# snap-research/MMVID

Measured on AMD Instinct MI355X. Metric: video-tokens/sec training step, 8-frame 128px text-to-video, higher is better.
Workload: dtype bf16

## Files before the change

include/mmvid_hip.h:

```cpp
#ifndef MMVID_HIP_H
#define MMVID_HIP_H
#include <stdint.h>
#ifdef __cplusplus
extern "C" {
#endif

const char* mmvid_last_error(void);
int mmvid_abi_version(void);
int mmvid_device_count(void);

int mmvid_vq_sqnorm(const float* codebook, int n, int dim, float* ee, void* stream);
int mmvid_vq_argmin_l2(const float* z, const float* codebook, const float* ee, int64_t rows, int n, int dim,
                       int64_t* idx, float* dmin, void* stream);
int mmvid_gather_rows(const float* table, int64_t table_rows, const int64_t* idx, int64_t rows, int dim,
                      float* out_f32, void* out_bf16, void* stream);

int mmvid_gemm_bf16(int a_kmajor, int b_kmajor, int M, int N, int K, const void* A, int64_t lda, const void* B,
                    int64_t ldb, int batch, int64_t strideA, int64_t strideB, int64_t strideC, int splitk,
                    float alpha, const float* bias, const float* residual, int64_t ldr, const void* dact_pre,
                    void* save_pre, int64_t ldp, int act, int accumulate, float* out_f32, void* out_bf16,
                    int64_t ldc, float* out_colsum,
                    void* stream);

int mmvid_decode_trace(void* dev_buf);
int mmvid_decode_persistent_trace(void* dev_buf);

int mmvid_gemm_bf16_dw(int64_t M, int N, int K, const void* dY, int64_t ldy, const void* X, int64_t ldx, int splitk,
                       float* workspace, float* dW, int accumulate, void* stream);
int mmvid_gemm_dw_pick_splitk(int64_t M, int N, int K);
typedef struct {
    int N, K;
    const void* dY;
    int64_t ldy, strideY;
    const void* X;
    int64_t ldx, strideX;
    float* const* dW_list;
} mmvid_dw_kind_t;
int mmvid_gemm_bf16_dw_multi(int64_t M, int nkinds, const mmvid_dw_kind_t* kinds, int groups, int accumulate, void* stream);
int mmvid_gemm_bf16_dw_grouped(int64_t M, int N, int K, const void* dY, int64_t ldy, int64_t strideY, const void* X, int64_t ldx,
                               int64_t strideX, int groups, float* const* dW_list, int accumulate, void* stream);
double mmvid_gemm_dw_multi_fill(int nkinds, const mmvid_dw_kind_t* kinds, int groups);

int mmvid_layernorm_fwd(const float* x, int64_t ldx, int64_t rows, int E, const float* w, const float* b, float eps,
                        void* y_bf16, float* y_f32, int64_t ldy, float* mean, float* rstd, void* stream);
int mmvid_layernorm_bwd(const float* dy, int64_t lddy, const float* x, int64_t ldx, const float* mean,
                        const float* rstd, const float* w, int64_t rows, int E, float* dx, int64_t lddx,
                        int add_into_dx, void* dx_bf16, float* dw, float* db, float* dx_colsum, void* stream);
int mmvid_layernorm_bwd_ws(const float* dy, int64_t lddy, const float* x, int64_t ldx, const float* mean,
                           const float* rstd, const float* w, int64_t rows, int E, float* dx, int64_t lddx,
                           int add_into_dx, void* dx_bf16, float* dw, float* db, float* dx_colsum, float* workspace,
                           int64_t workspace_floats, void* stream);
int mmvid_layernorm_bwd_ex(const void* dy, int dy_is_bf16, int64_t lddy, const float* x, int64_t ldx, const float* mean,
                           const float* rstd, const float* w, int64_t rows, int E, float* dx, int64_t lddx, int add_into_dx,
                           void* dx_bf16, float* dw, float* db, float* dx_colsum, float* workspace, int64_t workspace_floats,
                           void* stream);
typedef struct {
    const float* partial;
    float *dw, *db, *dx_colsum;
} mmvid_ln_reduce_t;
int mmvid_layernorm_bwd_partial(const void* dy, int dy_is_bf16, int64_t lddy, const float* x, int64_t ldx, const float* mean,
                                const float* rstd, const float* w, int64_t rows, int E, float* dx, int64_t lddx, int add_into_dx,
                                void* dx_bf16, int want_dw, int want_db, int want_colsum, float* workspace,
                                int64_t workspace_floats, int* blocks_out, void* stream);
int mmvid_layernorm_bwd_reduce_multi(int n, const mmvid_ln_reduce_t* items, int blocks, int E, void* stream);
int mmvid_groupnorm_swish_nhwc(const void* x, int x_is_bf16, int N, int64_t hw, int C, const float* w,
                               const float* b, float eps, int swish, float* stats_scratch, int partial_blocks,
                               void* y_bf16, float* y_f32, void* stream);

int mmvid_attention_fwd(const void* qkv, int64_t ld, int B, int L, int H, int E, float scale, int mask_mode, int r0,
                        int c0, int r1, int c1, void* out, int64_t ldo, float* lse2, void* stream);
int mmvid_attention_bwd(const void* qkv, int64_t ld, const void* O, int64_t ldo, const void* dO, int64_t lddo,
                        const float* lse2, float* delta, int B, int L, int H, int E, float scale, int mask_mode,
                        int r0, int c0, int r1, int c1, void* dqkv, int64_t ldg, void* stream);
int mmvid_attention_bwd_bias(const void* qkv, int64_t ld, const void* O, int64_t ldo, const void* dO, int64_t lddo,
// ... 342 lines not shown
```

mmvid_amd/_lib.py:

```python
import ctypes
import os
from ctypes import POINTER, Structure, c_char_p, c_float, c_int, c_int32, c_int64, c_uint8, c_uint64, c_void_p

HERE = os.path.dirname(os.path.abspath(__file__))
LIB_PATH = os.environ.get('MMVID_LIB') or os.path.join(HERE, 'libmmvid_hip.so')

P = c_void_p
I, I64, F, U64 = c_int, c_int64, c_float, c_uint64


class TowerLayer(Structure):
    _fields_ = [(n, P) for n in (
        'ln1_w', 'ln1_b', 'ln2_w', 'ln2_b', 'in_w', 'in_b', 'out_w', 'out_b', 'fc_w', 'fc_b', 'pj_w', 'pj_b',
        'g_ln1_w', 'g_ln1_b', 'g_ln2_w', 'g_ln2_b', 'g_in_w', 'g_in_b', 'g_out_w', 'g_out_b', 'g_fc_w', 'g_fc_b',
        'g_pj_w', 'g_pj_b')]


class TowerCfg(Structure):
    _fields_ = [('B', I), ('L', I), ('E', I), ('H', I), ('F', I), ('layers', I), ('mask_mode', I), ('r0', I),
                ('c0', I), ('r1', I), ('c1', I), ('ln_eps', F)]


class DecodeToken(Structure):
    _fields_ = [('tok', c_void_p), ('table', c_void_p), ('table_rows', c_int64), ('pos_rows', c_void_p), ('pos_off', c_int32),
# ... 1 lines not shown
                ('head_w', c_void_p), ('head_b', c_void_p), ('E', c_void_p), ('e_step_stride', c_int64), ('tok_offset', c_int64),
                ('logits_out', c_void_p), ('V', c_int32), ('e_pos0', c_int32), ('lnf_eps', c_float), ('temperature', c_float)]


class PostLnLayer(Structure):
    _fields_ = [(n, P) for n in ('qkv_w', 'qkv_b', 'out_w', 'out_b', 'ln1_w', 'ln1_b', 'fc_w', 'fc_b', 'pj_w', 'pj_b', 'ln2_w', 'ln2_b')]


class PostLnCfg(Structure):
    _fields_ = [('B', I), ('L', I), ('E', I), ('H', I), ('F', I), ('layers', I), ('ln_eps', F)]


class Conv3dCfg(Structure):
    _fields_ = [(n, I) for n in ('N', 'T', 'H', 'W', 'Cin', 'Cout', 'kt', 'kh', 'kw', 'st', 'sh', 'sw', 'pt0', 'pt1', 'ph0', 'ph1',
                                 'pw0', 'pw1', 'relu', 'nseg')] + [('seg_end', I * 3), ('ldo', I * 3), ('c_off', I * 3), ('out', P * 3)]


class VqganOp(Structure):
    _fields_ = [('op', c_int32), ('mode', c_int32), ('N', c_int32), ('H', c_int32), ('W', c_int32), ('C', c_int32),
                ('Cout', c_int32), ('flags', c_int32), ('in0', I64), ('in1', I64), ('in2', I64), ('out_bf16', I64),
                ('out_f32', I64), ('scratch', I64), ('w', P), ('b', P), ('ext_in', P), ('ext_out', P), ('eps', F),
                ('pad', c_int32)]


SIGNATURES = {
    'mmvid_vq_sqnorm': [P, I, I, P, P],
    'mmvid_vq_argmin_l2': [P, P, P, I64, I, I, P, P, P],
    'mmvid_gather_rows': [P, I64, P, I64, I, P, P, P],
    'mmvid_gemm_bf16': [I, I, I, I, I, P, I64, P, I64, I, I64, I64, I64, I, F, P, P, I64, P, P, I64, I, I, P, P, I64, P, P],
    'mmvid_gemm_bf16_dw': [I64, I, I, P, I64, P, I64, I, P, P, I, P],
    'mmvid_gemm_dw_pick_splitk': [I64, I, I],
    'mmvid_gemm_bf16_dw_grouped': [I64, I, I, P, I64, I64, P, I64, I64, I, P, I, P],
    'mmvid_gemm_bf16_dw_multi': [I64, I, P, I, I, P],
    'mmvid_layernorm_fwd': [P, I64, I64, I, P, P, F, P, P, I64, P, P, P],
    'mmvid_layernorm_bwd': [P, I64, P, I64, P, P, P, I64, I, P, I64, I, P, P, P, P, P],
    'mmvid_layernorm_bwd_ws': [P, I64, P, I64, P, P, P, I64, I, P, I64, I, P, P, P, P, P, I64, P],
    'mmvid_layernorm_bwd_partial': [P, I, I64, P, I64, P, P, P, I64, I, P, I64, I, P, I, I, I, P, I64, P, P],
    'mmvid_layernorm_bwd_reduce_multi': [I, P, I, I, P],
    'mmvid_layernorm_bwd_ex': [P, I, I64, P, I64, P, P, P, I64, I, P, I64, I, P, P, P, P, P, I64, P],
    'mmvid_groupnorm_swish_nhwc': [P, I, I, I64, I, P, P, F, I, P, I, P, P, P],
    'mmvid_attention_fwd': [P, I64, I, I, I, I, F, I, I, I, I, I, P, I64, P, P],
    'mmvid_attention_bwd': [P, I64, P, I64, P, I64, P, P, I, I, I, I, F, I, I, I, I, I, P, I64, P],
    'mmvid_attention_bwd_bias': [P, I64, P, I64, P, I64, P, P, I, I, I, I, F, I, I, I, I, I, P, I64, P, P],
    'mmvid_assemble_sequence': [POINTER(P), POINTER(I64), I, P, P, P, I64, I, I, P, P],
    'mmvid_assemble_sequence_bwd': [POINTER(P), POINTER(I64), I, P, P, P, I64, I, I, P, I, P],
    'mmvid_cross_entropy_fwd': [P, I64, P, P, I64, I, P, P, P],
    'mmvid_cross_entropy_bwd': [P, I64, P, P, P, P, I64, I, P, I64, P],
    'mmvid_colsum_bf16': [P, I64, I64, I, P, P],
    'mmvid_grad_sqnorm': [P, I64, P, P],
    'mmvid_adam_step': [P, P, P, P, P, I64, F, F, F, F, F, I, P, F, P, F, P],
    'mmvid_cast_f32_to_bf16': [P, P, I64, P],
    'mmvid_tower_workspace': [POINTER(TowerCfg), POINTER(I64), POINTER(I64)],
    'mmvid_tower_forward': [POINTER(TowerCfg), POINTER(TowerLayer), P, P, P, P, P],
    'mmvid_tower_backward': [POINTER(TowerCfg), POINTER(TowerLayer), P, P, P, P],
    'mmvid_tower_prefill': [POINTER(TowerCfg), POINTER(TowerLayer), P, P, P, I, P, P],
    'mmvid_tower_decode': [POINTER(TowerCfg), POINTER(TowerLayer), P, P, P, I, P, I, P, P],
    'mmvid_tower_decode_fused': [POINTER(TowerCfg), POINTER(TowerLayer), P, P, P, I, P, I, P, P],
    'mmvid_tower_decode_persistent': [POINTER(TowerCfg), POINTER(TowerLayer), P, P, P, I, P, I, I, P, P],
    'mmvid_artv_token_step_persistent': [POINTER(TowerCfg), POINTER(TowerLayer), POINTER(DecodeToken), P, P, I, P, P, P],
    'mmvid_tower_decode_fused_slice': [POINTER(TowerCfg), POINTER(TowerLayer), P, P, P, I, I, P, I, I, P, P],
    'mmvid_gemv_rows': [P, I64, I, I, P, P, F, P, P, I, I, P, I64, I, I, P, I64, P],
    'mmvid_decode_embed': [P, P, I64, P, P, I, I, I, P, P],
    'mmvid_decode_embed_record': [P, P, I64, P, P, I, I, I, P, P, I64, I, P],
    'mmvid_kv_store': [P, I64, I, I, I, P, I, I, P, P],
    'mmvid_attention_decode': [P, I64, P, I, I, I, I, P, I, F, P, I64, P],
    'mmvid_conv2d_nhwc': [I, P, I, I, I, I, P, P, I, P, P, I, P, P, P, P],
# ... 53 lines not shown
    'mmvid_get_option': [c_char_p, POINTER(I)],
    'mmvid_colsum_bf16_det': [P, I64, I64, I, P, P, I64, P],
    'mmvid_cross_entropy_fwd_det': [P, I64, P, P, I64, I, P, P, P, I64, P],
    'mmvid_assemble_sequence_bwd_det': [POINTER(P), POINTER(I64), I, P, P, P, I64, I, I, P, I, P, I64, P],
    'mmvid_gemm_bf16_det': [I, I, I, I, I, P, I64, P, I64, I, I64, I64, I64, I, F, P, P, I64, P, P, I64, I, I, P, P, I64, P, P, I64, P],
    'mmvid_attention_bwd_bias_det': [P, I64, P, I64, P, I64, P, P, I, I, I, I, F, I, I, I, I, I, P, I64, P, P, I64, P],
    'mmvid_device_faults': [P, I],
    'mmvid_pos_table_fwd': [P, I, I, I, P, P],
    'mmvid_pos_table_bwd': [P, I, I, P, P],
    'mmvid_lincomb3': [P, P, P, F, F, F, P, P],
    'mmvid_scale3': [P, F, F, F, P, P, P, P],
    'mmvid_prof_end': [P, P, P, P, I],
    'mmvid_rows_pack': [P, I64, I, P, I, P, P, P],
    'mmvid_rows_merge': [P, I64, I, P, P, I, P],
    'mmvid_clip_patchify': [P, I, I, I, I, I, P, P],
    'mmvid_clip_image_assemble': [P, P, P, P, P, F, I, I, I, P, P],
    'mmvid_clip_text_embed': [P, I, I, P, I64, P, I, P, P, P],
    'mmvid_clip_pool_project': [P, I, I, I, P, P, P, F, P, I, I, P, P],
    'mmvid_clip_pair_scores': [P, P, I, I, I, P, P],
    'mmvid_roberta_embed': [P, P, I, I, P, I64, P, I64, P, P, P, F, I, I64, P, P, P, P],
    'mmvid_attention_fwd_keylen': [P, I64, I, I, I, I, F, P, P, I64, P, P],
    'mmvid_postln_encoder_workspace': [POINTER(PostLnCfg), POINTER(I64)],
    'mmvid_postln_encoder_forward': [POINTER(PostLnCfg), POINTER(PostLnLayer), P, P, P, P, P, P],
    'mmvid_masked_mean_pool': [P, P, I, I, I, P, P],
    'mmvid_conv3d_ndhwc': [POINTER(Conv3dCfg), P, P, P, P],
    'mmvid_maxpool3d_ndhwc': [P, I, I, I, I, I, I, I, I, I, I, I, I, I, I, I, I, I, P, I, I, P],
    'mmvid_i3d_preprocess': [P, I, I, I, I, I, P, P],
    'mmvid_i3d_fold': [P, I, I, P, P],
    'mmvid_i3d_head': [P, I, I, I, P, P, I, P, P],
    'mmvid_frames_to_u8': [P, I64, I, I, P, P],
}
OTHER = {'mmvid_last_error': ([], c_char_p), 'mmvid_abi_version': ([], I), 'mmvid_device_count': ([], I),
         'mmvid_warp_params_bytes': ([], I), 'mmvid_gemm_dw_multi_fill': ([I, P, I], ctypes.c_double),
         'mmvid_tower_decode_persistent_supported': ([POINTER(TowerCfg), I], I),
         'mmvid_tower_decode_persistent_workspace_bytes': ([I], I64),
         'mmvid_colsum_bf16_det_workspace_bytes': ([I64, I], I64), 'mmvid_cross_entropy_fwd_det_workspace_bytes': ([I64], I64),
         'mmvid_assemble_sequence_bwd_det_workspace_bytes': ([I64, I, I, I, POINTER(I64)], I64),
         'mmvid_gemm_bf16_det_workspace_bytes': ([I, I, I, I], I64),
         'mmvid_attention_bwd_bias_det_workspace_bytes': ([I, I, I], I64)}

class DwKind(ctypes.Structure):
    _fields_ = [('N', ctypes.c_int32), ('K', ctypes.c_int32), ('dY', ctypes.c_void_p), ('ldy', ctypes.c_int64), ('strideY', ctypes.c_int64),
                ('X', ctypes.c_void_p), ('ldx', ctypes.c_int64), ('strideX', ctypes.c_int64), ('dW_list', ctypes.c_void_p)]


class LnReduce(ctypes.Structure):
    _fields_ = [('partial', ctypes.c_void_p), ('dw', ctypes.c_void_p), ('db', ctypes.c_void_p), ('dx_colsum', ctypes.c_void_p)]


class PosSegment(ctypes.Structure):
    _fields_ = [('w', ctypes.c_void_p * 3), ('gw', ctypes.c_void_p * 3), ('dst0', ctypes.c_int32), ('rows', ctypes.c_int32),
                ('naxes', ctypes.c_int32), ('src0', ctypes.c_int32), ('d', ctypes.c_int32 * 3), ('pad', ctypes.c_int32)]


ABI_VERSION = 3
_lib = None


class MMVIDError(RuntimeError):
    pass


def load():
    global _lib
    if _lib is None:
        import torch
# ... 81 lines not shown
```

mmvid_amd/csrc/common.h:

```cpp
#pragma once
#include <hip/hip_runtime.h>
#include <stdint.h>
#include <stdio.h>
#include <stdlib.h>
#include <string.h>

typedef uint16_t bf16_t;
typedef __attribute__((ext_vector_type(8))) __bf16 bf16x8_t;
typedef __attribute__((ext_vector_type(8))) _Float16 f16x8_t;
typedef __attribute__((ext_vector_type(4))) float f32x4;
typedef __attribute__((ext_vector_type(16))) float f32x16;

#define MMVID_OK 0
#define MMVID_ERR_ARG 1
#define MMVID_ERR_HIP 2

extern "C" const char* mmvid_last_error();
void mmvid_set_error(const char* fmt, ...);

#define MMVID_REQUIRE(cond, ...)          \
    do {                                  \
        if (!(cond)) {                    \
            mmvid_set_error(__VA_ARGS__); \
            return MMVID_ERR_ARG;         \
// ... 36 lines not shown
template <int CTRL>
__device__ __forceinline__ float dpp_mov(float v) {
    return __builtin_bit_cast(float, __builtin_amdgcn_update_dpp(0, __builtin_bit_cast(int, v), CTRL, 0xf, 0xf, true));
}
__device__ __forceinline__ float wave_sum_fast(float v) {
    v += dpp_mov<0xB1>(v);
    v += dpp_mov<0x4E>(v);
    v += dpp_mov<0x141>(v);
    v += dpp_mov<0x140>(v);
    const uint32_t u = __float_as_uint(v);
    const auto r = __builtin_amdgcn_permlane16_swap(u, u, false, false);
    v = __uint_as_float(r[0]) + __uint_as_float(r[1]);
    const uint32_t w = __float_as_uint(v);
    const auto q = __builtin_amdgcn_permlane32_swap(w, w, false, false);
    return __uint_as_float(q[0]) + __uint_as_float(q[1]);
}
__device__ __forceinline__ float wave_max_fast(float v) {
    v = fmaxf(v, dpp_mov<0xB1>(v));
    v = fmaxf(v, dpp_mov<0x4E>(v));
    v = fmaxf(v, dpp_mov<0x141>(v));
    v = fmaxf(v, dpp_mov<0x140>(v));
    const uint32_t u = __float_as_uint(v);
    const auto r = __builtin_amdgcn_permlane16_swap(u, u, false, false);
    v = fmaxf(__uint_as_float(r[0]), __uint_as_float(r[1]));
    const uint32_t w = __float_as_uint(v);
    const auto q = __builtin_amdgcn_permlane32_swap(w, w, false, false);
    return fmaxf(__uint_as_float(q[0]), __uint_as_float(q[1]));
}

__device__ __forceinline__ void mfma_settle(f32x16& acc) { asm volatile("s_nop 15" : "+v"(acc)); }
__device__ __forceinline__ void mfma_settle(f32x4& acc) { asm volatile("s_nop 15" : "+v"(acc)); }

static inline int cdiv(long a, long b) { return (int)((a + b - 1) / b); }
enum { MMVID_OPT_GRAPHS = 0, MMVID_OPT_DETERMINISTIC = 1, MMVID_OPT_COUNT = 2 };
int mmvid_option(int which);
int mmvid_slab_reduce(const float* slab, int nslabs, int N, float* out, hipStream_t stream);
unsigned long long* mmvid_fault_counters_dev();
```

mmvid_amd/csrc/errors.hip:

```cpp
#include <stdarg.h>

#include "common.h"

static thread_local char g_err[512] = "";

void mmvid_set_error(const char* fmt, ...) {
    va_list ap;
    va_start(ap, fmt);
    vsnprintf(g_err, sizeof(g_err), fmt, ap);
    va_end(ap);
}

extern "C" const char* mmvid_last_error() { return g_err; }

extern "C" int mmvid_abi_version() { return 3; }

extern "C" int mmvid_device_count() {
    int n = 0;
    if (hipGetDeviceCount(&n) != hipSuccess) return 0;
    return n;
}

namespace {
struct Opt {
    const char* name;
    const char* env;
    int dflt, value;
    bool set;
};
Opt g_opts[MMVID_OPT_COUNT] = {{"graphs", "MMVID_GRAPHS", 0, 0, false}, {"deterministic", "MMVID_DETERMINISTIC", 0, 0, false}};
}

int mmvid_option(int which) {
    Opt& o = g_opts[which];
    if (!o.set) {
        const char* e = getenv(o.env);
        o.value = e ? atoi(e) : o.dflt;
        o.set = true;
    }
    return o.value;
}

extern "C" int mmvid_set_option(const char* name, int value) {
    MMVID_REQUIRE(name, "set_option: null name");
    for (int i = 0; i < MMVID_OPT_COUNT; ++i)
        if (strcmp(name, g_opts[i].name) == 0) {
            g_opts[i].value = value, g_opts[i].set = true;
            return MMVID_OK;
        }
    mmvid_set_error("set_option: unknown option '%s' (graphs, deterministic)", name);
    return MMVID_ERR_ARG;
}

extern "C" int mmvid_get_option(const char* name, int* value) {
    MMVID_REQUIRE(name && value, "get_option: null pointer");
    for (int i = 0; i < MMVID_OPT_COUNT; ++i)
        if (strcmp(name, g_opts[i].name) == 0) {
            *value = mmvid_option(i);
            return MMVID_OK;
        }
    mmvid_set_error("get_option: unknown option '%s' (graphs, deterministic)", name);
    return MMVID_ERR_ARG;
}

#include <mutex>
#include <vector>

#include "graphs.h"
#include "prof.h"

namespace {
struct Rec {
    hipEvent_t a, b;
    int cls;
    double flops;
};
bool g_prof_on = false;
int g_prof_stride = 1;
int64_t g_prof_seen[PROF_NCLASS];
std::vector<Rec> g_recs;
std::vector<hipEvent_t> g_pool;
size_t g_pool_next = 0;
std::mutex g_prof_mu;

hipEvent_t pool_get() {
    if (g_pool_next == g_pool.size()) {
        hipEvent_t e;
        (void)hipEventCreate(&e);
        g_pool.push_back(e);
    }
    return g_pool[g_pool_next++];
}
}

// ... 53 lines not shown
```

mmvid_amd/csrc/gemm.hip:

```cpp
#include "../../include/mmvid_hip.h"
#include "gemm_core.h"
#include "prof.h"

namespace {
using namespace mmvid_core;


constexpr int GROUP_MAX = 48;
constexpr int KIND_MAX = 4;
struct GroupKind {
    const unsigned short* A;
    const unsigned short* B;
    long strideA, strideB, lda, ldb;
    int M, N, tiles_n, tiles_m;
    int first;
    int out0;
    int colmajor;
};

struct GemmParams {
    const bf16_t* A;
    const bf16_t* B;
    int M, N, K;
    long lda, ldb;
// ... 553 lines not shown
        tile_origin(tile, bm0, bn0);
        f32x16 acc[2][2];
#pragma unroll
        for (int i = 0; i < 2; ++i)
#pragma unroll
            for (int j = 0; j < 2; ++j)
#pragma unroll
                for (int r = 0; r < 16; ++r) acc[i][j][r] = 0.0f;
        [[maybe_unused]] PreRegs pre_in;
        if constexpr (EPI == 4) pre_load(p, de, bm0, bn0, wm, wn, lane, pre_in);
        k_loop_consumer<AKM, BKM>(smem, nt, wave, lane, wm, wn, acc);
        if constexpr (EPI == 4) {
            pending_fill_dact(p, pre_in, acc, pend, bm0, bn0, wm, wn, lane);
            pending_flush<1>(de, pend);
        } else if constexpr (EPI >= 2) {
            BiasRegs br;
            bias_load(bias_lds, bn0, wn, lane, br);
            pending_fill<NOUT>(p, br, acc, pend, bm0, bn0, wm, wn, lane);
            pending_flush<NOUT>(de, pend);
        } else {
            gemm_epilogue_direct(p, de, bias_lds, acc, bm0, bn0, wm, wn, lane);
        }
    }
}

template <bool AKM, bool BKM, int EPI>
__global__ __launch_bounds__(512 + 64 * mmvid_core::NLOAD, 1) void gemm_bf16_lw_kernel(GemmParams p) {
    gemm_lw_body<AKM, BKM, EPI, false>(p, nullptr);
}
__global__ __launch_bounds__(512 + 64 * mmvid_core::NLOAD, 1) void gemm_bf16_lw_grouped_kernel(GemmParams p, GroupTable gt) {
    gemm_lw_body<true, true, 1, true>(p, &gt);
}

__global__ __launch_bounds__(256) void splitk_reduce_kernel(const float* __restrict__ partial, int splitk, long mn,
                                                            float* __restrict__ out, int accumulate) {
    const long i = ((long)blockIdx.x * 256 + threadIdx.x) * 4;
    if (i >= mn) return;
    float4 a = accumulate ? *reinterpret_cast<const float4*>(out + i) : make_float4(0, 0, 0, 0);
    for (int s = 0; s < splitk; ++s) {
        const float4 v = *reinterpret_cast<const float4*>(partial + (long)s * mn + i);
        a.x += v.x, a.y += v.y, a.z += v.z, a.w += v.w;
    }
    *reinterpret_cast<float4*>(out + i) = a;
}

bool use_big_tile(long M, long N, long zdim) {
    const long blocks = (long)cdiv(M, 256) * cdiv(N, BN) * zdim;
    return M >= 256 && blocks >= 200;
}

constexpr int BIAS_LDS_BYTES = 16384;
bool direct_epilogue_ok(const GemmParams& p) {
    if (p.splitk != 1 || p.partial || p.colsum || p.N > BIAS_LDS_BYTES / 4) return false;
    const long rows = p.M - 1;
    const long ld = p.ldc > p.ldp ? p.ldc : p.ldp;
    const long ldr = p.residual ? p.ldr : 0;
    return (rows * (ld > ldr ? ld : ldr) + p.N) * 4 < (1ll << 31);
}

template <bool AKM, bool BKM, int WM>
void launch_shape(const GemmParams& p, int batch, hipStream_t stream) {
    using S = BlockShape<WM>;
    dim3 grid(cdiv(p.N, BN), cdiv(p.M, S::ROWS), batch * p.splitk);
    GemmParams q = p;
    q.tiles_n = q.tiles_m = 0;
    q.group_n = 0;
// ... 247 lines not shown
        p.A = gt.kinds[0].A, p.B = gt.kinds[0].B;
        p.M = gt.kinds[0].M, p.N = gt.kinds[0].N, p.K = (int)M, p.lda = gt.kinds[0].lda, p.ldb = gt.kinds[0].ldb;
        p.strideA = p.strideB = p.strideC = 0, p.splitk = 1;
        p.bias = nullptr, p.residual = nullptr, p.ldr = 0, p.dact_pre = nullptr, p.save_pre = nullptr, p.ldp = 0;
        p.act = 0, p.accumulate = accumulate, p.alpha = 1.0f;
        p.out_f32 = nullptr, p.out_bf16 = nullptr, p.ldc = gt.kinds[0].N;
        p.partial = nullptr, p.colsum = nullptr, p.colsum_det = 0;
        p.tiles_n = p.tiles_m = 0, p.group_n = 0;
        MmvidProfScope prof(PROF_GEMM_TN, flops, (hipStream_t)stream);
        hipLaunchKernelGGL(gemm_bf16_lw_grouped_kernel, dim3(tiles), dim3(512 + 64 * NLOAD), S::LDS_BYTES + BIAS_LDS_BYTES, (hipStream_t)stream, p, gt);
    }
    MMVID_LAUNCH_CHECK("gemm_bf16_dw_multi");
    return MMVID_OK;
}

extern "C" int mmvid_gemm_bf16_dw_grouped(int64_t M, int N, int K, const void* dY, int64_t ldy, int64_t strideY, const void* X,
                                          int64_t ldx, int64_t strideX, int groups, float* const* dW_list, int accumulate,
                                          void* stream) {
    mmvid_dw_kind_t kd;
    kd.N = N, kd.K = K, kd.dY = dY, kd.ldy = ldy, kd.strideY = strideY, kd.X = X, kd.ldx = ldx, kd.strideX = strideX, kd.dW_list = dW_list;
    return mmvid_gemm_bf16_dw_multi(M, 1, &kd, groups, accumulate, stream);
}

extern "C" double mmvid_gemm_dw_multi_fill(int nkinds, const mmvid_dw_kind_t* kinds, int groups) {
    long tiles = 0;
    for (int k = 0; k < nkinds; ++k) {
        long live = 0;
        for (int g = 0; g < groups; ++g) live += kinds[k].dW_list == nullptr || kinds[k].dW_list[g] != nullptr;
        tiles += (long)cdiv(kinds[k].N, 256) * cdiv(kinds[k].K, BN) * live;
    }
    const long rounds = cdiv(tiles, 256);
    return tiles > 0 ? (double)tiles / (double)(rounds * 256) : 0.0;
}
```

mmvid_amd/csrc/tower.hip:

```cpp
#include "../../include/mmvid_hip.h"
#include "common.h"
#include <vector>

#include "graphs.h"

namespace {

inline int64_t align256(int64_t x) { return (x + 255) & ~(int64_t)255; }
constexpr int kMaxSplitK = 16;
constexpr int kLnBwdBlocks = 512;

struct Dims {
    int B, L, E, H, F, layers;
    int64_t M;
};
Dims dims_of(const mmvid_tower_cfg_t& c) {
    Dims d;
    d.B = c.B, d.L = c.L, d.E = c.E, d.H = c.H, d.F = c.F, d.layers = c.layers;
    d.M = (int64_t)c.B * c.L;
    return d;
}

struct SavedLayer {
    int64_t x_in, x_mid, mean1, rstd1, mean2, rstd2, h1, qkv, o, lse2, h2, pre, act, k_gpj, k_dpre, k_gout, k_dqkv, k_ln1, k_ln2, total;
// ... 140 lines not shown
            }
            x = xin_s;
        }
        float* xnext;
        if (i == d.layers - 1)
            xnext = x_out;
        else if (saved)
            xnext = (float*)((char*)saved + (int64_t)(i + 1) * sl.total + sl.x_in);
        else
            xnext = x_out;
        TRY(mmvid_layernorm_fwd(x, d.E, d.M, d.E, ly.ln1_w, ly.ln1_b, cfg->ln_eps, sv + sl.h1, nullptr, d.E,
                                (float*)(sv + sl.mean1), (float*)(sv + sl.rstd1), stream));
        TRY(linear_fwd(d.M, 3 * d.E, d.E, sv + sl.h1, ly.in_w, ly.in_b, nullptr, nullptr, 0, nullptr, sv + sl.qkv, stream));
        if (kv_cache)
            TRY(mmvid_kv_store(sv + sl.qkv, 3 * d.E, d.B, d.L, d.E, nullptr, 0, kv_lmax,
                               (char*)kv_cache + (int64_t)i * d.B * kv_lmax * 2 * d.E * 2, stream));
        TRY(mmvid_attention_fwd(sv + sl.qkv, 3 * d.E, d.B, d.L, d.H, d.E, scale, cfg->mask_mode, cfg->r0, cfg->c0, cfg->r1,
                                cfg->c1, sv + sl.o, d.E, (float*)(sv + sl.lse2), stream));
        TRY(linear_fwd(d.M, d.E, d.E, sv + sl.o, ly.out_w, ly.out_b, x, nullptr, 0, xmid, nullptr, stream));
        TRY(mmvid_layernorm_fwd(xmid, d.E, d.M, d.E, ly.ln2_w, ly.ln2_b, cfg->ln_eps, sv + sl.h2, nullptr, d.E,
                                (float*)(sv + sl.mean2), (float*)(sv + sl.rstd2), stream));
        TRY(linear_fwd(d.M, d.F, d.E, sv + sl.h2, ly.fc_w, ly.fc_b, nullptr, saved ? sv + sl.pre : nullptr, 1, nullptr,
                       sv + sl.act, stream));
        TRY(linear_fwd(d.M, d.E, d.F, sv + sl.act, ly.pj_w, ly.pj_b, xmid, nullptr, 0, xnext, nullptr, stream));
        x = xnext;
    }
    return MMVID_OK;
}

extern "C" int mmvid_tower_backward(const mmvid_tower_cfg_t* cfg, const mmvid_tower_layer_t* layers, float* g,
                                    void* saved, void* scratch, void* stream) {
    TRY(check_cfg(cfg));
    MMVID_REQUIRE(layers && g && saved && scratch, "tower_backward: null pointer");
    const uint64_t key = tower_key(mmvid_option(MMVID_OPT_DETERMINISTIC) ? 5 : 3, cfg, layers, g, saved, scratch, nullptr, stream);
    return mmvid_run_cached(key, (hipStream_t)stream, [=](hipStream_t s) {
        return tower_backward_enqueue(cfg, layers, g, saved, scratch, (void*)s);
    });
}

static int tower_backward_enqueue(const mmvid_tower_cfg_t* cfg, const mmvid_tower_layer_t* layers, float* g, void* saved,
                                  void* scratch, void* stream) {
    const Dims d = dims_of(*cfg);
    const SavedLayer sl = saved_layout(d);
    const Scratch sc = scratch_layout(d);
    char* scr = (char*)scratch;
    char* keep = (char*)saved;
    struct { int64_t g_pj, d_pre, g_out, dqkv, total; } kl = {sl.k_gpj, sl.k_dpre, sl.k_gout, sl.k_dqkv, sl.total};
    const float scale = 0.125f;
    void* d_h = scr + sc.d_h;
    float* ws = (float*)(scr + sc.splitk_ws);
    void* det_ws = nullptr;
    const int64_t det_bytes = det_slab_bytes(d);
    if (mmvid_option(MMVID_OPT_DETERMINISTIC)) {
        MMVID_REQUIRE(det_bytes <= sc.total - sc.infer, "tower_backward: the deterministic slabs do not fit the scratch arena");
        det_ws = scr + sc.infer;
    }
    const int64_t ln_ws_floats = (int64_t)kLnBwdBlocks * 3 * d.E;
    std::vector<mmvid_ln_reduce_t> ln_items;
    int ln_blocks = 0;
    for (int i = d.layers - 1; i >= 0; --i) {
        const mmvid_tower_layer_t& ly = layers[i];
        const char* sv = (const char*)saved + (int64_t)i * sl.total;
        char* kp = keep + (int64_t)i * kl.total;
        void* g_pj = kp + kl.g_pj;
        if (i == d.layers - 1) {
            TRY(mmvid_cast_f32_to_bf16(g, g_pj, d.M * d.E, stream));
            if (ly.g_pj_b && det_ws) TRY(mmvid_colsum_bf16_det(g_pj, d.E, d.M, d.E, ly.g_pj_b, det_ws, det_bytes, stream));
// ... 24 lines not shown
            int nb = 0;
            TRY(mmvid_layernorm_bwd_partial(d_h, 1, d.E, (const float*)(sv + sl.x_in), d.E, (const float*)(sv + sl.mean1),
                                            (const float*)(sv + sl.rstd1), ly.ln1_w, d.M, d.E, g, d.E, 1,
                                            i > 0 ? (void*)(keep + (int64_t)(i - 1) * kl.total + kl.g_pj) : nullptr, r.dw != nullptr,
                                            r.db != nullptr, r.dx_colsum != nullptr, (float*)(kp + sl.k_ln1), ln_ws_floats, &nb, stream));
            if (r.dw || r.db || r.dx_colsum) ln_items.push_back(r), ln_blocks = nb;
        }
    }
    if (!ln_items.empty()) TRY(mmvid_layernorm_bwd_reduce_multi((int)ln_items.size(), ln_items.data(), ln_blocks, d.E, stream));
    struct Kind {
        int N, K;
        int64_t dy_off, x_off;
        float* mmvid_tower_layer_t::*gw;
    };
    const Kind kinds[4] = {{d.E, d.F, kl.g_pj, sl.act, &mmvid_tower_layer_t::g_pj_w},
                           {d.F, d.E, kl.d_pre, sl.h2, &mmvid_tower_layer_t::g_fc_w},
                           {d.E, d.E, kl.g_out, sl.o, &mmvid_tower_layer_t::g_out_w},
                           {3 * d.E, d.E, kl.dqkv, sl.h1, &mmvid_tower_layer_t::g_in_w}};
    std::vector<float*> outs((size_t)d.layers * 4);
    mmvid_dw_kind_t kd[4];
    int nk = 0;
    for (const Kind& k : kinds) {
        float** o = outs.data() + (size_t)nk * d.layers;
        bool any = false;
        for (int i = 0; i < d.layers; ++i) o[i] = layers[i].*(k.gw), any = any || o[i];
        if (!any) continue;
        kd[nk].N = k.N, kd[nk].K = k.K;
        kd[nk].dY = keep + k.dy_off, kd[nk].ldy = k.N, kd[nk].strideY = kl.total / 2;
        kd[nk].X = (const char*)saved + k.x_off, kd[nk].ldx = k.K, kd[nk].strideX = sl.total / 2;
        kd[nk].dW_list = o;
        ++nk;
    }
    if (nk == 0) return MMVID_OK;
    if (mmvid_gemm_dw_multi_fill(nk, kd, d.layers) >= 0.7) return mmvid_gemm_bf16_dw_multi(d.M, nk, kd, d.layers, 1, stream);
    for (int k = 0; k < nk; ++k)
        for (int i = d.layers - 1; i >= 0; --i)
            TRY(linear_dw(d.M, kd[k].N, kd[k].K, (const char*)kd[k].dY + (int64_t)i * kl.total, (const char*)kd[k].X + (int64_t)i * sl.total,
                          kd[k].dW_list[i], nullptr, ws, stream));
    return MMVID_OK;
}

extern "C" int mmvid_tower_prefill(const mmvid_tower_cfg_t* cfg, const mmvid_tower_layer_t* layers, const float* x_in,
                                   float* x_out, void* kv_cache, int Lmax, void* scratch, void* stream) {
    TRY(check_cfg(cfg));
    MMVID_REQUIRE(layers && x_in && x_out && kv_cache && scratch, "tower_prefill: null pointer");
    MMVID_REQUIRE(cfg->mask_mode == 1 && cfg->L <= Lmax, "tower_prefill: needs the causal mask and L (%d) <= Lmax (%d)", cfg->L,
                  Lmax);
    return tower_forward_enqueue(cfg, layers, x_in, x_out, nullptr, scratch, stream, kv_cache, Lmax);
}

extern "C" int mmvid_tower_decode(const mmvid_tower_cfg_t* cfg, const mmvid_tower_layer_t* layers, const float* x_in,
                                  float* x_out, void* kv_cache, int Lmax, const int32_t* pos_dev, int pos, void* scratch,
                                  void* stream) {
    TRY(check_cfg(cfg));
    MMVID_REQUIRE(layers && x_in && x_out && kv_cache && scratch, "tower_decode: null pointer");
    MMVID_REQUIRE(cfg->mask_mode == 1, "tower_decode: incremental decoding needs the causal mask");
    const int B = cfg->B, E = cfg->E, F = cfg->F, H = cfg->H;
    char* p = (char*)scratch;
    auto take = [&](int64_t bytes) {
        char* o = p;
        p += align256(bytes);
        return o;
    };
    void* h = take((int64_t)B * E * 2);
    void* qkv = take((int64_t)B * 3 * E * 2);
    void* o = take((int64_t)B * E * 2);
    float* xmid = (float*)take((int64_t)B * E * 4);
// ... 21 lines not shown
```

mmvid_amd/ops.py:

```python
import ctypes

import torch

from . import _lib
from ._lib import call

bf16, f32, i64 = torch.bfloat16, torch.float32, torch.int64


def _stream():
    return ctypes.c_void_p(torch.cuda.current_stream().cuda_stream)


def _p(t):
    if t is None:
        return None
    return ctypes.c_void_p(t.data_ptr())


_DET_WS = {}


def _det_ws(op, device, nbytes):
    key = (op, str(device), int(nbytes))
# ... 123 lines not shown
    return dW


def gemm_dw_grouped(dY, X, dWs, accumulate=True):
    _chk(dY, bf16, 'dY'), _chk(X, bf16, 'X')
    G, M, N = dY.shape
    K = X.shape[2]
    assert X.shape[:2] == (G, M) and len(dWs) == G
    ptrs = (ctypes.c_void_p * G)(*[(_chk(w, f32, 'dW').data_ptr() if w is not None else None) for w in dWs])
    call('mmvid_gemm_bf16_dw_grouped', M, N, K, _p(dY), dY.stride(1), dY.stride(0), _p(X), X.stride(1), X.stride(0), G, ptrs,
         int(accumulate), _stream())
    return dWs


def _dw_kinds(kinds):
    arr = (_lib.DwKind * len(kinds))()
    keep = []
    G, M = kinds[0][0].shape[:2]
    for a, (dY, X, dWs) in zip(arr, kinds):
        _chk(dY, bf16, 'dY'), _chk(X, bf16, 'X')
        assert dY.shape[:2] == (G, M) and X.shape[:2] == (G, M) and len(dWs) == G
        ptrs = (ctypes.c_void_p * G)(*[(_chk(w, f32, 'dW').data_ptr() if w is not None else None) for w in dWs])
        keep.append(ptrs)
        a.N, a.K, a.dY, a.ldy, a.strideY = dY.shape[2], X.shape[2], dY.data_ptr(), dY.stride(1), dY.stride(0)
        a.X, a.ldx, a.strideX, a.dW_list = X.data_ptr(), X.stride(1), X.stride(0), ctypes.cast(ptrs, ctypes.c_void_p)
    return arr, keep, M, G


def gemm_dw_multi(kinds, accumulate=True):
    arr, keep, M, G = _dw_kinds(kinds)
    call('mmvid_gemm_bf16_dw_multi', M, len(kinds), arr, G, int(accumulate), _stream())


def gemm_dw_multi_fill(shapes, groups):
    arr = (_lib.DwKind * len(shapes))()
    for a, (N, K) in zip(arr, shapes):
        a.N, a.K, a.dW_list = N, K, None
    return _lib.load().mmvid_gemm_dw_multi_fill(len(shapes), arr, groups)


def gemm_f32(A, B, *, b_kmajor=False, bias=None, residual=None, alpha=1.0):
    _chk(A, f32, 'A'), _chk(B, f32, 'B')
    M, K = A.shape
    N = B.shape[1] if b_kmajor else B.shape[0]
    out = torch.empty(M, N, device=A.device, dtype=f32)
    call('mmvid_gemm_f32', int(b_kmajor), M, N, K, _p(A), K, _p(B), B.shape[1], 1, 0, 0, 0, float(alpha), _p(bias),
         _p(residual), _p(out), N, _stream())
    return out


def layernorm_fwd(x, w, b, eps=1e-5, out_dtype=bf16, save_stats=True):
    _chk(x, f32, 'x')
    rows, E = x.numel() // x.shape[-1], x.shape[-1]
    y = torch.empty(x.shape, device=x.device, dtype=out_dtype)
    mean = torch.empty(rows, device=x.device, dtype=f32) if save_stats else None
    rstd = torch.empty(rows, device=x.device, dtype=f32) if save_stats else None
    call('mmvid_layernorm_fwd', _p(x), E, rows, E, _p(w), _p(b), float(eps), _p(y) if out_dtype == bf16 else None,
         _p(y) if out_dtype == f32 else None, E, _p(mean), _p(rstd), _stream())
    return y, mean, rstd


def layernorm_bwd(dy, x, mean, rstd, w, dx=None, add=False, dw=None, db=None, dx_colsum=None, workspace=None):
    _chk(dy, f32, 'dy'), _chk(x, f32, 'x')
    rows, E = x.numel() // x.shape[-1], x.shape[-1]
    if dx is None:
        dx = torch.empty_like(x)
# ... 417 lines not shown
```

Measured before the change: 210,900.

## Add balanced stream-K schedule for grouped weight-gradient GEMM in tower backward

Adds a persistent 256-block grouped dW GEMM kernel that runs full output tiles in rounds and splits the leftover tail tiles along K evenly across all blocks, ordered by XCD. Partial tiles go to workspace slabs and a fixup kernel sums them into dW. The tower backward uses this path by default when the scratch has room. It targets wave-quantization idle time in the last round, at the cost of an extra reduction kernel and workspace traffic.

```diff
diff --git a/include/mmvid_hip.h b/include/mmvid_hip.h
--- a/include/mmvid_hip.h
+++ b/include/mmvid_hip.h
@@ -40,6 +40,12 @@
 int mmvid_gemm_bf16_dw_grouped(int64_t M, int N, int K, const void* dY, int64_t ldy, int64_t strideY, const void* X, int64_t ldx,
                                int64_t strideX, int groups, float* const* dW_list, int accumulate, void* stream);
 double mmvid_gemm_dw_multi_fill(int nkinds, const mmvid_dw_kind_t* kinds, int groups);
+int mmvid_gemm_bf16_dw_multi_ws(int64_t M, int nkinds, const mmvid_dw_kind_t* kinds, int groups, int accumulate, void* workspace,
+                                int64_t workspace_bytes, void* stream);
+int64_t mmvid_gemm_bf16_dw_multi_ws_workspace_bytes(int64_t M, int nkinds, const mmvid_dw_kind_t* kinds, int groups);
+int mmvid_gemm_dw_multi_plan(int tiles, int ktiles, int block, int* items, int max_items);
+int mmvid_gemm_dw_multi_plan_blocks(void);
+int64_t mmvid_gemm_dw_multi_plan_workspace_bytes(int tiles, int ktiles);
 
 int mmvid_layernorm_fwd(const float* x, int64_t ldx, int64_t rows, int E, const float* w, const float* b, float eps,
                         void* y_bf16, float* y_f32, int64_t ldy, float* mean, float* rstd, void* stream);
diff --git a/mmvid_amd/_lib.py b/mmvid_amd/_lib.py
--- a/mmvid_amd/_lib.py
+++ b/mmvid_amd/_lib.py
@@ -57,6 +57,7 @@
     'mmvid_gemm_dw_pick_splitk': [I64, I, I],
     'mmvid_gemm_bf16_dw_grouped': [I64, I, I, P, I64, I64, P, I64, I64, I, P, I, P],
     'mmvid_gemm_bf16_dw_multi': [I64, I, P, I, I, P],
+    'mmvid_gemm_bf16_dw_multi_ws': [I64, I, P, I, I, P, I64, P],
     'mmvid_layernorm_fwd': [P, I64, I64, I, P, P, F, P, P, I64, P, P, P],
     'mmvid_layernorm_bwd': [P, I64, P, I64, P, P, P, I64, I, P, I64, I, P, P, P, P, P],
     'mmvid_layernorm_bwd_ws': [P, I64, P, I64, P, P, P, I64, I, P, I64, I, P, P, P, P, P, I64, P],
@@ -176,6 +177,8 @@
 }
 OTHER = {'mmvid_last_error': ([], c_char_p), 'mmvid_abi_version': ([], I), 'mmvid_device_count': ([], I),
          'mmvid_warp_params_bytes': ([], I), 'mmvid_gemm_dw_multi_fill': ([I, P, I], ctypes.c_double),
+         'mmvid_gemm_bf16_dw_multi_ws_workspace_bytes': ([I64, I, P, I], I64), 'mmvid_gemm_dw_multi_plan': ([I, I, I, P, I], I),
+         'mmvid_gemm_dw_multi_plan_blocks': ([], I), 'mmvid_gemm_dw_multi_plan_workspace_bytes': ([I, I], I64),
          'mmvid_tower_decode_persistent_supported': ([POINTER(TowerCfg), I], I),
          'mmvid_tower_decode_persistent_workspace_bytes': ([I], I64),
          'mmvid_colsum_bf16_det_workspace_bytes': ([I64, I], I64), 'mmvid_cross_entropy_fwd_det_workspace_bytes': ([I64], I64),
diff --git a/mmvid_amd/csrc/common.h b/mmvid_amd/csrc/common.h
--- a/mmvid_amd/csrc/common.h
+++ b/mmvid_amd/csrc/common.h
@@ -92,7 +92,7 @@
 __device__ __forceinline__ void mfma_settle(f32x4& acc) { asm volatile("s_nop 15" : "+v"(acc)); }
 
 static inline int cdiv(long a, long b) { return (int)((a + b - 1) / b); }
-enum { MMVID_OPT_GRAPHS = 0, MMVID_OPT_DETERMINISTIC = 1, MMVID_OPT_COUNT = 2 };
+enum { MMVID_OPT_GRAPHS = 0, MMVID_OPT_DETERMINISTIC = 1, MMVID_OPT_DW_BALANCED = 2, MMVID_OPT_COUNT = 3 };
 int mmvid_option(int which);
 int mmvid_slab_reduce(const float* slab, int nslabs, int N, float* out, hipStream_t stream);
 unsigned long long* mmvid_fault_counters_dev();
diff --git a/mmvid_amd/csrc/errors.hip b/mmvid_amd/csrc/errors.hip
--- a/mmvid_amd/csrc/errors.hip
+++ b/mmvid_amd/csrc/errors.hip
@@ -28,7 +28,8 @@
     int dflt, value;
     bool set;
 };
-Opt g_opts[MMVID_OPT_COUNT] = {{"graphs", "MMVID_GRAPHS", 0, 0, false}, {"deterministic", "MMVID_DETERMINISTIC", 0, 0, false}};
+Opt g_opts[MMVID_OPT_COUNT] = {{"graphs", "MMVID_GRAPHS", 0, 0, false}, {"deterministic", "MMVID_DETERMINISTIC", 0, 0, false},
+                               {"dw_balanced", "MMVID_DW_BALANCED", 1, 1, false}};
 }
 
 int mmvid_option(int which) {
@@ -48,7 +49,7 @@
             g_opts[i].value = value, g_opts[i].set = true;
             return MMVID_OK;
         }
-    mmvid_set_error("set_option: unknown option '%s' (graphs, deterministic)", name);
+    mmvid_set_error("set_option: unknown option '%s' (graphs, deterministic, dw_balanced)", name);
     return MMVID_ERR_ARG;
 }
 
@@ -59,7 +60,7 @@
             *value = mmvid_option(i);
             return MMVID_OK;
         }
-    mmvid_set_error("get_option: unknown option '%s' (graphs, deterministic)", name);
+    mmvid_set_error("get_option: unknown option '%s' (graphs, deterministic, dw_balanced)", name);
     return MMVID_ERR_ARG;
 }
 
diff --git a/mmvid_amd/csrc/gemm.hip b/mmvid_amd/csrc/gemm.hip
--- a/mmvid_amd/csrc/gemm.hip
+++ b/mmvid_amd/csrc/gemm.hip
@@ -609,6 +609,180 @@
     gemm_lw_body<true, true, 1, true>(p, &gt);
 }
 
+constexpr int DW_BLOCKS = 256;
+constexpr int DW_SLAB = 256 * 128;
+struct DwPlan {
+    int T, nk;
+    int rounds, full, R;
+    int q, r;
+};
+struct DwItem {
+    int tile, kt0, nt;
+    int slab;
+};
+__host__ __device__ inline DwPlan dw_plan(int T, int nk) {
+    DwPlan pl;
+    pl.T = T, pl.nk = nk;
+    pl.rounds = T / DW_BLOCKS, pl.full = pl.rounds * DW_BLOCKS, pl.R = T - pl.full;
+    const int U = pl.R * nk;
+    pl.q = U / DW_BLOCKS, pl.r = U - pl.q * DW_BLOCKS;
+    return pl;
+}
+__host__ __device__ inline int dw_xcd_order(int id, int n) {
+    const int xcd = id & 7, q = n >> 3, r = n & 7;
+    return (xcd < r ? xcd * (q + 1) : r * (q + 1) + (xcd - r) * q) + (id >> 3);
+}
+__host__ __device__ inline int dw_share_start(const DwPlan& pl, int s) { return s * pl.q + (s < pl.r ? s : pl.r); }
+__host__ __device__ inline int dw_share_of(const DwPlan& pl, int u) {
+    const int big = pl.r * (pl.q + 1);
+    return u < big ? u / (pl.q + 1) : pl.r + (u - big) / pl.q;
+}
+__host__ __device__ inline int dw_item_count(const DwPlan& pl, int b) {
+    const int s = dw_xcd_order(b, DW_BLOCKS);
+    const int u0 = dw_share_start(pl, s), u1 = dw_share_start(pl, s + 1);
+    if (u1 == u0) return pl.rounds;
+    return pl.rounds + (u1 > (u0 / pl.nk + 1) * pl.nk ? 2 : 1);
+}
+__host__ __device__ inline DwItem dw_item(const DwPlan& pl, int b, int i) {
+    DwItem it;
+    if (i < pl.rounds) {
+        it.tile = dw_xcd_order(b + i * DW_BLOCKS, pl.full), it.kt0 = 0, it.nt = pl.nk, it.slab = -1;
+        return it;
+    }
+    const int s = dw_xcd_order(b, DW_BLOCKS);
+    const int u0 = dw_share_start(pl, s), u1 = dw_share_start(pl, s + 1);
+    const int t0 = u0 / pl.nk;
+    const bool two = u1 > (t0 + 1) * pl.nk;
+    if ((i == pl.rounds) != two) {
+        const int end = u1 < (t0 + 1) * pl.nk ? u1 : (t0 + 1) * pl.nk;
+        it.tile = pl.full + t0, it.kt0 = u0 - t0 * pl.nk, it.nt = end - u0;
+        it.slab = it.nt == pl.nk ? -1 : s + t0;
+    } else {
+        it.tile = pl.full + t0 + 1, it.kt0 = 0, it.nt = u1 - (t0 + 1) * pl.nk;
+        it.slab = it.nt == pl.nk ? -1 : s + t0 + 1;
+    }
+    return it;
+}
+inline int dw_plan_slabs(const DwPlan& pl) {
+    int n = 0;
+    for (int b = 0; b < DW_BLOCKS; ++b)
+        for (int i = pl.rounds, e = dw_item_count(pl, b); i < e; ++i) {
+            const DwItem it = dw_item(pl, b, i);
+            if (it.slab >= n) n = it.slab + 1;
+        }
+    return n;
+}
+
+struct DwTable {
+    GroupTable gt;
+    unsigned char grp[GROUP_MAX];
+    int T, nk;
+    int tokens;
+    int accumulate;
+    float* ws;
+};
+struct DwTile {
+    const bf16_t *A, *B;
+    long lda, ldb;
+    int M, N, bm0, bn0;
+    float* out;
+};
+__device__ __forceinline__ DwTile dw_tile(const DwTable& tb, int wg) {
+    using S = BlockShape<4>;
+    GroupKind kd = tb.gt.kinds[0];
+#pragma unroll
+    for (int i = 1; i < KIND_MAX; ++i)
+        if (wg >= tb.gt.kinds[i].first) kd = tb.gt.kinds[i];
+    const int rem = wg - kd.first, per = kd.tiles_n * kd.tiles_m;
+    const int slot = rem / per, t = rem - slot * per;
+    const int g = tb.grp[kd.out0 + slot];
+    int tm, tn;
+    if (kd.colmajor)
+        tn = t / kd.tiles_m, tm = t - tn * kd.tiles_m;
+    else
+        tm = t / kd.tiles_n, tn = t - tm * kd.tiles_n;
+    DwTile o;
+    o.A = kd.A + (long)g * kd.strideA, o.B = kd.B + (long)g * kd.strideB;
+    o.lda = kd.lda, o.ldb = kd.ldb, o.M = kd.M, o.N = kd.N;
+    o.bm0 = tm * S::ROWS, o.bn0 = tn * BN;
+    o.out = tb.gt.out_list[kd.out0 + slot];
+    return o;
+}
+
+__global__ __launch_bounds__(512 + 64 * mmvid_core::NLOAD, 1) void gemm_bf16_lw_grouped_balanced_kernel(DwTable tb) {
+    constexpr int NMW = 8, NL = NLOAD;
+    extern __shared__ __attribute__((aligned(16))) char smem[];
+    const int tid = threadIdx.x;
+    const int lane = tid & 63, wave = __builtin_amdgcn_readfirstlane(tid >> 6);
+    const int wm = (wave & 7) >> 1, wn = wave & 1;
+    const DwPlan pl = dw_plan(tb.T, tb.nk);
+    const int b = blockIdx.x;
+    const int n_items = dw_item_count(pl, b);
+    const int K = tb.tokens;
+    if (wave >= NMW) {
+        const int w = wave - NMW;
+        LoaderStage<true, NL> sa;
+        LoaderStage<true, NL> sb;
+        DwItem it;
+        auto start = [&](int i) {
+            it = dw_item(pl, b, i);
+            const DwTile t = dw_tile(tb, it.tile);
+            sa.init(t.A, t.lda, t.M, K, t.bm0), sb.init(t.B, t.ldb, t.N, K, t.bn0), sa.init_offsets(2, w, lane), sb.init_offsets(1, w, lane);
+            loader_prologue<true, true, NL>(sa, sb, smem, it.kt0, it.nt, K, w, lane);
+        };
+        if (n_items > 0) start(0);
+        for (int i = 0; i < n_items; ++i) {
+            k_loop_loader<true, true, NL>(sa, sb, smem, it.kt0, it.nt, K, w, lane);
+            if (i + 1 < n_items) start(i + 1);
+        }
+        return;
+    }
+    for (int i = 0; i < n_items; ++i) {
+        const DwItem it = dw_item(pl, b, i);
+        const DwTile t = dw_tile(tb, it.tile);
+        const bool whole = it.slab < 0;
+        GemmParams p;
+        p.A = nullptr, p.B = nullptr, p.K = K, p.lda = p.ldb = 0, p.strideA = p.strideB = p.strideC = 0, p.splitk = 1;
+        p.bias = nullptr, p.residual = nullptr, p.ldr = 0, p.dact_pre = nullptr, p.save_pre = nullptr, p.ldp = 0;
+        p.act = 0, p.alpha = 1.0f, p.out_bf16 = nullptr, p.partial = nullptr, p.colsum = nullptr, p.colsum_det = 0;
+        p.tiles_n = p.tiles_m = 0, p.group_n = 0;
+        p.M = whole ? t.M : 256, p.N = whole ? t.N : BN, p.ldc = p.N;
+        p.out_f32 = whole ? t.out : tb.ws + (long)it.slab * DW_SLAB;
+        p.accumulate = whole ? tb.accumulate : 0;
+        DirectEpi de;
+        de.init(p, 0);
+        f32x16 acc[2][2];
+#pragma unroll
+        for (int ii = 0; ii < 2; ++ii)
+#pragma unroll
+            for (int j = 0; j < 2; ++j)
+#pragma unroll
+                for (int r = 0; r < 16; ++r) acc[ii][j][r] = 0.0f;
+        k_loop_consumer<true, true>(smem, it.nt, wave, lane, wm, wn, acc);
+        gemm_epilogue_direct(p, de, nullptr, acc, whole ? t.bm0 : 0, whole ? t.bn0 : 0, wm, wn, lane);
+    }
+}
+
+__global__ __launch_bounds__(256) void dw_fixup_kernel(DwTable tb) {
+    const DwPlan pl = dw_plan(tb.T, tb.nk);
+    const int t = blockIdx.y;
+    const int s0 = dw_share_of(pl, t * pl.nk), s1 = dw_share_of(pl, (t + 1) * pl.nk - 1);
+    if (s0 == s1) return;
+    const DwTile tl = dw_tile(tb, pl.full + t);
+    for (int e = blockIdx.x * 256 + threadIdx.x; e < DW_SLAB / 4; e += gridDim.x * 256) {
+        const int row = e >> 5, c = (e & 31) * 4;
+        const int m = tl.bm0 + row, n = tl.bn0 + c;
+        if (m >= tl.M || n >= tl.N) continue;
+        float* o = tl.out + (long)m * tl.N + n;
+        float4 a = tb.accumulate ? *reinterpret_cast<const float4*>(o) : make_float4(0.f, 0.f, 0.f, 0.f);
+        for (int s = s0; s <= s1; ++s) {
+            const float4 v = *reinterpret_cast<const float4*>(tb.ws + (long)(s + t) * DW_SLAB + row * BN + c);
+            a.x += v.x, a.y += v.y, a.z += v.z, a.w += v.w;
+        }
+        *reinterpret_cast<float4*>(o) = a;
+    }
+}
+
 __global__ __launch_bounds__(256) void splitk_reduce_kernel(const float* __restrict__ partial, int splitk, long mn,
                                                             float* __restrict__ out, int accumulate) {
     const long i = ((long)blockIdx.x * 256 + threadIdx.x) * 4;
@@ -922,3 +1096,101 @@
     const long rounds = cdiv(tiles, 256);
     return tiles > 0 ? (double)tiles / (double)(rounds * 256) : 0.0;
 }
+
+namespace {
+int dw_live_tiles(const mmvid_dw_kind_t* kinds, int nkinds, int g0, int n) {
+    long tiles = 0;
+    for (int k = 0; k < nkinds; ++k) {
+        int live = 0;
+        for (int g = 0; g < n; ++g) live += kinds[k].dW_list[g0 + g] != nullptr;
+        tiles += (long)cdiv(kinds[k].N, 256) * cdiv(kinds[k].K, BN) * live;
+    }
+    return tiles < (1l << 30) ? (int)tiles : -1;
+}
+}
+
+extern "C" int mmvid_gemm_dw_multi_plan(int tiles, int ktiles, int block, int* items, int max_items) {
+    if (tiles < 0 || ktiles <= 0 || ktiles > (1 << 22) || block < 0 || block >= DW_BLOCKS || (max_items > 0 && !items)) return -1;
+    const DwPlan pl = dw_plan(tiles, ktiles);
+    const int n = dw_item_count(pl, block);
+    for (int i = 0; i < n && i < max_items; ++i) {
+        const DwItem it = dw_item(pl, block, i);
+        items[4 * i] = it.tile, items[4 * i + 1] = it.kt0, items[4 * i + 2] = it.nt, items[4 * i + 3] = it.slab;
+    }
+    return n;
+}
+extern "C" int mmvid_gemm_dw_multi_plan_blocks(void) { return DW_BLOCKS; }
+extern "C" int64_t mmvid_gemm_dw_multi_plan_workspace_bytes(int tiles, int ktiles) {
+    if (tiles < 0 || ktiles <= 0 || ktiles > (1 << 22)) return -1;
+    return (int64_t)dw_plan_slabs(dw_plan(tiles, ktiles)) * DW_SLAB * 4;
+}
+extern "C" int64_t mmvid_gemm_bf16_dw_multi_ws_workspace_bytes(int64_t M, int nkinds, const mmvid_dw_kind_t* kinds, int groups) {
+    if (!kinds || M <= 0 || nkinds <= 0 || nkinds > KIND_MAX || groups <= 0 || cdiv(M, (int64_t)BK) > (1 << 22)) return -1;
+    for (int k = 0; k < nkinds; ++k)
+        if (!kinds[k].dW_list || kinds[k].N <= 0 || kinds[k].K <= 0) return -1;
+    const int per_launch = GROUP_MAX / nkinds;
+    int64_t need = 0;
+    for (int g0 = 0; g0 < groups; g0 += per_launch) {
+        const int T = dw_live_tiles(kinds, nkinds, g0, groups - g0 < per_launch ? groups - g0 : per_launch);
+        if (T < 0) return -1;
+        const int64_t b = mmvid_gemm_dw_multi_plan_workspace_bytes(T, (int)cdiv(M, (int64_t)BK));
+        if (b > need) need = b;
+    }
+    return need;
+}
+
+extern "C" int mmvid_gemm_bf16_dw_multi_ws(int64_t M, int nkinds, const mmvid_dw_kind_t* kinds, int groups, int accumulate,
+                                           void* workspace, int64_t workspace_bytes, void* stream) {
+    MMVID_REQUIRE(kinds && M > 0 && nkinds > 0 && nkinds <= KIND_MAX && groups > 0, "gemm_bf16_dw_multi_ws: bad arguments");
+    MMVID_REQUIRE(cdiv(M, (int64_t)BK) <= (1 << 22), "gemm_bf16_dw_multi_ws: M too large");
+    using S = BlockShape<4>;
+    for (int k = 0; k < nkinds; ++k) {
+        const mmvid_dw_kind_t& kd = kinds[k];
+        MMVID_REQUIRE(kd.dY && kd.X && kd.dW_list && kd.N > 0 && kd.K > 0, "gemm_bf16_dw_multi_ws: kind %d: null pointer / bad size", k);
+        MMVID_REQUIRE(kd.N % 8 == 0 && kd.K % 8 == 0 && kd.ldy % 8 == 0 && kd.ldx % 8 == 0 && kd.strideY % 8 == 0 && kd.strideX % 8 == 0,
+                      "gemm_bf16_dw_multi_ws: kind %d: N, K, ldy, ldx and the group strides must be multiples of 8", k);
+        MMVID_REQUIRE(kd.ldy >= kd.N && kd.ldx >= kd.K, "gemm_bf16_dw_multi_ws: kind %d: ldy < N or ldx < K", k);
+        MMVID_REQUIRE(M * kd.ldy * 2 < (1ll << 31) && M * kd.ldx * 2 < (1ll << 31), "gemm_bf16_dw_multi_ws: an operand of 2 GiB or more per group");
+        MMVID_REQUIRE((int64_t)kd.N * kd.K < (1ll << 29), "gemm_bf16_dw_multi_ws: an output of 2 GiB or more");
+    }
+    const int64_t need = mmvid_gemm_bf16_dw_multi_ws_workspace_bytes(M, nkinds, kinds, groups);
+    MMVID_REQUIRE(need >= 0, "gemm_bf16_dw_multi_ws: too many output tiles");
+    MMVID_REQUIRE(need == 0 || (workspace && workspace_bytes >= need && ((uintptr_t)workspace & 15) == 0),
+                  "gemm_bf16_dw_multi_ws: a 16-byte aligned workspace of %lld bytes is needed (mmvid_gemm_bf16_dw_multi_ws_workspace_bytes)",
+                  (long long)need);
+    const int nk = (int)cdiv(M, (int64_t)BK);
+    const int per_launch = GROUP_MAX / nkinds;
+    for (int g0 = 0; g0 < groups; g0 += per_launch) {
+        const int n = groups - g0 < per_launch ? groups - g0 : per_launch;
+        DwTable tb;
+        GroupTable& gt = tb.gt;
+        gt.n_kinds = nkinds;
+        int tiles = 0, slots = 0;
+        double flops = 0;
+        for (int g = 0; g < GROUP_MAX; ++g) gt.out_list[g] = nullptr, tb.grp[g] = 0;
+        for (int k = 0; k < nkinds; ++k) {
+            GroupKind& o = gt.kinds[k];
+            const mmvid_dw_kind_t& kd = kinds[k];
+            o.A = (const unsigned short*)kd.dY + (int64_t)g0 * kd.strideY, o.B = (const unsigned short*)kd.X + (int64_t)g0 * kd.strideX;
+            o.strideA = kd.strideY, o.strideB = kd.strideX, o.lda = kd.ldy, o.ldb = kd.ldx;
+            o.M = kd.N, o.N = kd.K, o.tiles_n = cdiv(kd.K, BN), o.tiles_m = cdiv(kd.N, S::ROWS);
+            o.first = tiles, o.out0 = slots;
+            o.colmajor = kd.K > kd.N ? 1 : 0;
+            for (int g = 0; g < n; ++g) {
+                if (!kd.dW_list[g0 + g]) continue;
+                gt.out_list[slots] = kd.dW_list[g0 + g], tb.grp[slots] = (unsigned char)g;
+                ++slots, tiles += o.tiles_n * o.tiles_m, flops += 2.0 * M * kd.N * (double)kd.K;
+            }
+        }
+        for (int k = nkinds; k < KIND_MAX; ++k) gt.kinds[k] = gt.kinds[0], gt.kinds[k].first = 0x7fffffff;
+        if (tiles == 0) continue;
+        tb.T = tiles, tb.nk = nk, tb.tokens = (int)M, tb.accumulate = accumulate, tb.ws = (float*)workspace;
+        const DwPlan pl = dw_plan(tiles, nk);
+        MmvidProfScope prof(PROF_GEMM_TN, flops, (hipStream_t)stream);
+        (void)hipFuncSetAttribute((const void*)gemm_bf16_lw_grouped_balanced_kernel, hipFuncAttributeMaxDynamicSharedMemorySize, (int)S::LDS_BYTES);
+        hipLaunchKernelGGL(gemm_bf16_lw_grouped_balanced_kernel, dim3(DW_BLOCKS), dim3(512 + 64 * NLOAD), S::LDS_BYTES, (hipStream_t)stream, tb);
+        if (dw_plan_slabs(pl) > 0) hipLaunchKernelGGL(dw_fixup_kernel, dim3(8, pl.R), dim3(256), 0, (hipStream_t)stream, tb);
+    }
+    MMVID_LAUNCH_CHECK("gemm_bf16_dw_multi_ws");
+    return MMVID_OK;
+}
diff --git a/mmvid_amd/csrc/tower.hip b/mmvid_amd/csrc/tower.hip
--- a/mmvid_amd/csrc/tower.hip
+++ b/mmvid_amd/csrc/tower.hip
@@ -196,7 +196,7 @@
                                     void* saved, void* scratch, void* stream) {
     TRY(check_cfg(cfg));
     MMVID_REQUIRE(layers && g && saved && scratch, "tower_backward: null pointer");
-    const uint64_t key = tower_key(mmvid_option(MMVID_OPT_DETERMINISTIC) ? 5 : 3, cfg, layers, g, saved, scratch, nullptr, stream);
+    const uint64_t key = tower_key((mmvid_option(MMVID_OPT_DETERMINISTIC) ? 5 : 3) + (mmvid_option(MMVID_OPT_DW_BALANCED) ? 0 : 16), cfg, layers, g, saved, scratch, nullptr, stream);
     return mmvid_run_cached(key, (hipStream_t)stream, [=](hipStream_t s) {
         return tower_backward_enqueue(cfg, layers, g, saved, scratch, (void*)s);
     });
@@ -287,7 +287,12 @@
         ++nk;
     }
     if (nk == 0) return MMVID_OK;
-    if (mmvid_gemm_dw_multi_fill(nk, kd, d.layers) >= 0.7) return mmvid_gemm_bf16_dw_multi(d.M, nk, kd, d.layers, 1, stream);
+    if (mmvid_gemm_dw_multi_fill(nk, kd, d.layers) >= 0.7) {
+        const int64_t ws_bytes = sc.infer - sc.splitk_ws;
+        const int64_t need = mmvid_gemm_bf16_dw_multi_ws_workspace_bytes(d.M, nk, kd, d.layers);
+        if (mmvid_option(MMVID_OPT_DW_BALANCED) && need >= 0 && need <= ws_bytes) return mmvid_gemm_bf16_dw_multi_ws(d.M, nk, kd, d.layers, 1, ws, ws_bytes, stream);
+        return mmvid_gemm_bf16_dw_multi(d.M, nk, kd, d.layers, 1, stream);
+    }
     for (int k = 0; k < nk; ++k)
         for (int i = d.layers - 1; i >= 0; --i)
             TRY(linear_dw(d.M, kd[k].N, kd[k].K, (const char*)kd[k].dY + (int64_t)i * kl.total, (const char*)kd[k].X + (int64_t)i * sl.total,
diff --git a/mmvid_amd/ops.py b/mmvid_amd/ops.py
--- a/mmvid_amd/ops.py
+++ b/mmvid_amd/ops.py
@@ -179,6 +179,32 @@
     call('mmvid_gemm_bf16_dw_multi', M, len(kinds), arr, G, int(accumulate), _stream())
 
 
+def gemm_dw_multi_ws(kinds, accumulate=True, workspace=None):
+    arr, keep, M, G = _dw_kinds(kinds)
+    if workspace is None:
+        workspace = torch.empty(max(16, gemm_dw_multi_ws_bytes(kinds)), device=kinds[0][0].device, dtype=torch.uint8)
+    call('mmvid_gemm_bf16_dw_multi_ws', M, len(kinds), arr, G, int(accumulate), _p(workspace), workspace.numel() * workspace.element_size(),
+         _stream())
+
+
+def gemm_dw_multi_ws_bytes(kinds):
+    arr, keep, M, G = _dw_kinds(kinds)
+    return _lib.load().mmvid_gemm_bf16_dw_multi_ws_workspace_bytes(M, len(kinds), arr, G)
+
+
+def gemm_dw_multi_plan(tiles, ktiles):
+    lib = _lib.load()
+    cap = tiles // lib.mmvid_gemm_dw_multi_plan_blocks() + 2
+    buf = (ctypes.c_int32 * (4 * cap))()
+    plan = []
+    for b in range(lib.mmvid_gemm_dw_multi_plan_blocks()):
+        n = lib.mmvid_gemm_dw_multi_plan(tiles, ktiles, b, buf, cap)
+        if n < 0 or n > cap:
+            raise _lib.MMVIDError(f'mmvid_gemm_dw_multi_plan({tiles}, {ktiles}, {b}) returned {n}')
+        plan.append([tuple(buf[4 * i:4 * i + 4]) for i in range(n)])
+    return plan
+
+
 def gemm_dw_multi_fill(shapes, groups):
     arr = (_lib.DwKind * len(shapes))()
     for a, (N, K) in zip(arr, shapes):
```

Result: no change. 212,600, median of 6 (+0.8%).
